# sparsemat/sprs

Hardware: NVIDIA H100
Metric: csr_spmv_f64_gflops (higher is better)
Workload: dtype f64

## Files before the change

sprs_b200/csrc/api.cu:

```cuda

#include <algorithm>
#include <mutex>
#include <vector>

#include <cstdlib>

#include "common.cuh"
#include "ptx.cuh"

namespace {

__global__ void make_policies_kernel(uint64_t* out) {
    out[0] = policy_evict_first();
    out[1] = policy_evict_last();
}

thread_local std::string g_create_error;

template <typename Src, typename Dst>
__global__ void convert_rebase_kernel(const Src* __restrict__ in, Dst* __restrict__ out,
                                      uint64_t n, uint64_t base) {
    const uint64_t i = blockIdx.x * (uint64_t)blockDim.x + threadIdx.x;
    if (i < n) out[i] = (Dst)((uint64_t)in[i] - base);
}
// ... 303 lines not shown
        }
        if ((st = upload_indexlike(ctx, indptr, indptr_bytes, outer + 1, base, m->d_indptr,
                                   m->indptr_bytes, s)) != SPRS_B200_OK)
            break;
        if ((st = upload_indexlike(ctx, indices, index_bytes, nnz, 0, m->d_indices, 4, s)) !=
            SPRS_B200_OK)
            break;
        if (nnz > 0) {
            e = cudaMemcpyAsync(m->d_data, data, nnz * sizeof(double), cudaMemcpyHostToDevice, s);
            if (e != cudaSuccess) {
                sprs_b200_set_error(ctx, cudaGetErrorString(e));
                st = SPRS_B200_ERR_CUDA;
                break;
            }
        }
        if ((st = spmv_prepare(ctx, m, s)) != SPRS_B200_OK) break;
        e = cudaStreamSynchronize(s);
        if (e != cudaSuccess) {
            sprs_b200_set_error(ctx, cudaGetErrorString(e));
            st = SPRS_B200_ERR_CUDA;
        }
    } while (0);
    if (st != SPRS_B200_OK) {
        sprs_b200_csmat_free(m);
        return st;
    }
    *out = m;
    return SPRS_B200_OK;
}

int sprs_b200_csmat_from_device(sprs_b200_ctx* ctx, int storage, uint64_t rows, uint64_t cols,
                                uint64_t nnz, const uint32_t* d_indptr,
                                const uint32_t* d_indices, const double* d_data,
                                sprs_b200_csmat** out) {
    if (!ctx || !out || !d_indptr) return SPRS_B200_ERR_ARGUMENT;
    *out = nullptr;
    if (nnz >= 0xffffffffull || rows > 0xffffffffull || cols > 0xffffffffull)
        SPRS_FAIL(ctx, SPRS_B200_ERR_INDEX_RANGE, "from_device takes u32 arrays only");
    if (((uintptr_t)d_indices | (uintptr_t)d_data) & 15)
        SPRS_FAIL(ctx, SPRS_B200_ERR_ARGUMENT, "device arrays must be 16-byte aligned");
    SPRS_CUDA(ctx, cudaSetDevice(ctx->device));
    auto* m = new sprs_b200_csmat();
    m->ctx = ctx;
    m->storage = storage;
    m->rows = rows;
    m->cols = cols;
    m->nnz = nnz;
    m->outer = storage == SPRS_B200_CSR ? rows : cols;
    m->inner = storage == SPRS_B200_CSR ? cols : rows;
    m->indptr_bytes = 4;
    m->d_indptr = const_cast<uint32_t*>(d_indptr);
    m->d_indices = const_cast<uint32_t*>(d_indices);
    m->d_data = const_cast<double*>(d_data);
    m->owns = false;
    int st = spmv_prepare(ctx, m, ctx->stream);
    if (st == SPRS_B200_OK && cudaStreamSynchronize(ctx->stream) != cudaSuccess) {
        sprs_b200_set_error(ctx, "from_device: partition kernel failed");
        st = SPRS_B200_ERR_CUDA;
    }
    if (st != SPRS_B200_OK) {
        sprs_b200_csmat_free(m);
        return st;
    }
    *out = m;
    return SPRS_B200_OK;
}

int sprs_b200_csmat_free(sprs_b200_csmat* m) {
    if (!m) return SPRS_B200_OK;
    if (m->ctx) cudaSetDevice(m->ctx->device);
    if (m->owns && m->pooled && m->ctx) {
        cudaDeviceSynchronize();
        if (m->d_indptr) cudaFreeAsync(m->d_indptr, m->ctx->stream);
        if (m->d_indices) cudaFreeAsync(m->d_indices, m->ctx->stream);
        if (m->d_data) cudaFreeAsync(m->d_data, m->ctx->stream);
    } else if (m->owns) {
        if (m->d_indptr) cudaFree(m->d_indptr);
        if (m->d_indices) cudaFree(m->d_indices);
        if (m->d_data) cudaFree(m->d_data);
    }
    if (m->d_tile_row) cudaFree(m->d_tile_row);
    if (m->d_tile_k) cudaFree(m->d_tile_k);
    if (m->d_carry) cudaFree(m->d_carry);
    if (m->csr_cache) sprs_b200_csmat_free(m->csr_cache);
    delete m;
    return SPRS_B200_OK;
}

static int csr_of(sprs_b200_ctx* ctx, const sprs_b200_csmat* m, const sprs_b200_csmat** out) {
    if (m->storage == SPRS_B200_CSR) {
        *out = m;
        return SPRS_B200_OK;
    }
    if (!m->csr_cache) {
        sprs_b200_csmat* t = nullptr;
        SPRS_TRY(sprs_b200_csmat_to_other_storage(ctx, m, &t));
        m->csr_cache = t;
    }
    *out = m->csr_cache;
    return SPRS_B200_OK;
}

int sprs_b200_csmat_storage(const sprs_b200_csmat* m) { return m ? m->storage : -1; }
uint64_t sprs_b200_csmat_rows(const sprs_b200_csmat* m) { return m ? m->rows : 0; }
uint64_t sprs_b200_csmat_cols(const sprs_b200_csmat* m) { return m ? m->cols : 0; }
uint64_t sprs_b200_csmat_nnz(const sprs_b200_csmat* m) { return m ? m->nnz : 0; }

int sprs_b200_csmat_download(sprs_b200_ctx* ctx, const sprs_b200_csmat* m, void* indptr,
                             int indptr_bytes, void* indices, int index_bytes, double* data) {
    if (!ctx || !m || !indptr) return SPRS_B200_ERR_ARGUMENT;
    if ((indptr_bytes != 4 && indptr_bytes != 8) || (index_bytes != 4 && index_bytes != 8))
        SPRS_FAIL(ctx, SPRS_B200_ERR_ARGUMENT, "bad index width");
    if (indptr_bytes == 4 && m->nnz > 0xffffffffull)
        SPRS_FAIL(ctx, SPRS_B200_ERR_INDEX_RANGE, "Index type is not large enough for nnz");
    SPRS_CUDA(ctx, cudaSetDevice(ctx->device));
    cudaStream_t s = ctx->stream;
    SPRS_TRY(download_indexlike(ctx, m->d_indptr, m->indptr_bytes, m->outer + 1, indptr,
                                indptr_bytes, s));
    if (m->nnz) {
        if (!indices || !data) return SPRS_B200_ERR_ARGUMENT;
        SPRS_TRY(download_indexlike(ctx, m->d_indices, 4, m->nnz, indices, index_bytes, s));
        SPRS_CUDA(ctx, cudaMemcpyAsync(data, m->d_data, m->nnz * sizeof(double),
                                       cudaMemcpyDeviceToHost, s));
        SPRS_CUDA(ctx, cudaStreamSynchronize(s));
    }
    return SPRS_B200_OK;
}

int sprs_b200_csmat_device_arrays(const sprs_b200_csmat* m, const void** d_indptr,
                                  int* indptr_bytes, const uint32_t** d_indices,
                                  const double** d_data) {
    if (!m) return SPRS_B200_ERR_ARGUMENT;
    if (d_indptr) *d_indptr = m->d_indptr;
    if (indptr_bytes) *indptr_bytes = m->indptr_bytes;
    if (d_indices) *d_indices = m->d_indices;
    if (d_data) *d_data = m->d_data;
    return SPRS_B200_OK;
}

static int finish_triplets(sprs_b200_ctx* ctx, sprs_b200_csmat* t, int st, sprs_b200_csmat** out) {
    if (st == SPRS_B200_OK) st = spmv_prepare(ctx, t, ctx->stream);
    if (st == SPRS_B200_OK && cudaStreamSynchronize(ctx->stream) != cudaSuccess) {
        sprs_b200_set_error(ctx, "from_triplets: kernel failed");
        st = SPRS_B200_ERR_CUDA;
    }
    if (st != SPRS_B200_OK) {
        sprs_b200_csmat_free(t);
        return st;
    }
    *out = t;
    return SPRS_B200_OK;
}

int sprs_b200_csmat_from_triplets_dev(sprs_b200_ctx* ctx, uint64_t rows, uint64_t cols,
                                      uint64_t n, const uint32_t* d_row, const uint32_t* d_col,
                                      const double* d_val, sprs_b200_csmat** out) {
    if (!ctx || !out || (n && (!d_row || !d_col || !d_val))) return SPRS_B200_ERR_ARGUMENT;
    *out = nullptr;
    SPRS_CUDA(ctx, cudaSetDevice(ctx->device));
    auto* t = new sprs_b200_csmat();
    return finish_triplets(ctx, t, triplets_to_csr_launch(ctx, rows, cols, n, d_row, d_col, d_val,
                                                         t, ctx->stream), out);
}

int sprs_b200_csmat_from_triplets(sprs_b200_ctx* ctx, uint64_t rows, uint64_t cols, uint64_t n,
                                  const void* row_inds, const void* col_inds, int index_bytes,
// ... 318 lines not shown
```

sprs_b200/csrc/common.cuh:

```cuda
#pragma once
#include <cuda_runtime.h>

#include <cstdint>
#include <cstdio>
#include <cstring>
#include <string>
#include <vector>

#include "../../include/sprs_b200.h"

constexpr int SPRS_E2E_MAX_CHUNKS = 8;
constexpr int SPRS_E2E_DEFAULT_CHUNKS = 8;

struct sprs_b200_ctx {
    int device = 0;
    int sm_count = 132;
    size_t l2_bytes = 0;
    cudaStream_t stream = nullptr;
    std::string last_error;
    uint64_t launches = 0;
    uint64_t pol_evict_first = 0, pol_evict_last = 0;
    void* h_stage = nullptr;
    size_t h_stage_bytes = 0;
    void* d_scratch[4] = {nullptr, nullptr, nullptr, nullptr};
    size_t d_scratch_bytes[4] = {0, 0, 0, 0};
    cudaStream_t side_stream = nullptr;
    cudaEvent_t ev_fork = nullptr, ev_join = nullptr;
    cudaStream_t copy_stream = nullptr;
    cudaEvent_t ev_chunk[SPRS_E2E_MAX_CHUNKS] = {};
    cudaEvent_t ev_copied = nullptr;
};

struct sprs_b200_csmat {
    sprs_b200_ctx* ctx = nullptr;
    int storage = SPRS_B200_CSR;
    uint64_t rows = 0, cols = 0, nnz = 0;
    uint64_t outer = 0, inner = 0;
    int indptr_bytes = 4;
    void* d_indptr = nullptr;
    uint32_t* d_indices = nullptr;
    double* d_data = nullptr;
    bool owns = true;
    bool pooled = false;
    uint32_t* d_tile_row = nullptr;
    void* d_tile_k = nullptr;
    double* d_carry = nullptr;
    uint64_t n_tiles = 0;
    mutable sprs_b200_csmat* csr_cache = nullptr;
    mutable std::vector<uint64_t> e2e_tiles, e2e_rows;
    mutable std::vector<uint64_t> push_tiles, push_rows;
};

#define SPRS_FAIL(ctx, code, ...)                                  \
    do {                                                           \
        char _buf[512];                                            \
        snprintf(_buf, sizeof(_buf), __VA_ARGS__);                 \
        sprs_b200_set_error((ctx), _buf);                          \
        return (code);                                             \
    } while (0)

#define SPRS_CUDA(ctx, expr)                                                              \
    do {                                                                                  \
        cudaError_t _e = (expr);                                                          \
        if (_e != cudaSuccess)                                                            \
            SPRS_FAIL((ctx), SPRS_B200_ERR_CUDA, "%s failed: %s (%s:%d)", #expr,          \
                      cudaGetErrorString(_e), __FILE__, __LINE__);                        \
    } while (0)

#define SPRS_TRY(expr)                      \
    do {                                    \
        int _s = (expr);                    \
        if (_s != SPRS_B200_OK) return _s;  \
    } while (0)

void sprs_b200_set_error(const sprs_b200_ctx* ctx, const char* msg);

static inline cudaStream_t pick_stream(sprs_b200_ctx*, void* stream) {
    return (cudaStream_t)stream;
}

int ctx_scratch(sprs_b200_ctx* ctx, int i, size_t bytes, void** out);
int ctx_stage(sprs_b200_ctx* ctx, size_t bytes, void** out);

constexpr int SPMV_MAX_TARGETS = 8;
struct SpmvTargets {
    double* p[SPMV_MAX_TARGETS];
    int n;
};

int spmv_prepare(sprs_b200_ctx* ctx, sprs_b200_csmat* m, cudaStream_t s);
int spmv_tile_nnz();
int spmv_launch(sprs_b200_ctx* ctx, const sprs_b200_csmat* m, const double* d_x, double* d_y,
                int accumulate, cudaStream_t s);
int spmv_launch_targets(sprs_b200_ctx* ctx, const sprs_b200_csmat* m, const double* d_x,
                        const SpmvTargets& yt, int accumulate, cudaStream_t s);
int spmv_launch_tile_range(sprs_b200_ctx* ctx, const sprs_b200_csmat* m, const double* d_x,
                           double* d_y, int accumulate, uint64_t t0, uint64_t t1, cudaStream_t s);
int csmat_chunk_table(sprs_b200_ctx* ctx, const sprs_b200_csmat* m, uint64_t n_chunks, bool taper,
                      cudaStream_t s, std::vector<uint64_t>* tiles, std::vector<uint64_t>* rows);
int ctx_side_stream(sprs_b200_ctx* ctx);
int peer_push_launch(sprs_b200_ctx* ctx, const double* src, const SpmvTargets& dst, uint64_t count,
                     cudaStream_t s);
int spmm_rowmaj_launch(sprs_b200_ctx* ctx, const sprs_b200_csmat* m, const double* d_b,
                       uint64_t ldb, uint64_t k, double* d_c, uint64_t ldc, int accumulate,
                       cudaStream_t s);
int triplets_to_csr_launch(sprs_b200_ctx* ctx, uint64_t rows, uint64_t cols, uint64_t n,
                           const uint32_t* d_row, const uint32_t* d_col, const double* d_val,
                           sprs_b200_csmat* out, cudaStream_t s);
int transpose_launch(sprs_b200_ctx* ctx, const sprs_b200_csmat* m, sprs_b200_csmat* out,
                     cudaStream_t s);
int csmat_csr_view(sprs_b200_ctx* ctx, const sprs_b200_csmat* m, const sprs_b200_csmat** out);

#ifdef __CUDACC__
__device__ __forceinline__ uint32_t smem_u32(const void* p) {
    return (uint32_t)__cvta_generic_to_shared(p);
}
__device__ __forceinline__ uint64_t mix64(uint64_t z) {
    z += 0x9E3779B97F4A7C15ull;
    z = (z ^ (z >> 30)) * 0xBF58476D1CE4E5B9ull;
    z = (z ^ (z >> 27)) * 0x94D049BB133111EBull;
    return z ^ (z >> 31);
}
#endif
```

sprs_b200/csrc/spgemm.cu:

```cuda

#include <cstdlib>
#include <vector>

#include "common.cuh"
#include "scan.cuh"

struct sprs_b200_spgemm {
    sprs_b200_ctx* ctx = nullptr;
    const sprs_b200_csmat* a = nullptr;
    const sprs_b200_csmat* b = nullptr;
    uint64_t rows = 0, cols = 0, nnz_c = 0, n_prod = 0;
    uint64_t* d_nprod = nullptr;
    uint32_t* d_cnt = nullptr;
    uint64_t* d_cptr = nullptr;
    uint32_t* d_lists = nullptr;
    uint32_t* d_counters = nullptr;
};

namespace {

constexpr uint32_t EMPTY = 0xffffffffu;
constexpr int NT = 256;
constexpr int WARPS = NT / 32;
constexpr uint32_t SYM_S_MAX = 128, SYM_M_MAX = 8192;
// ... 757 lines not shown
            break;
        }
        const uint32_t *l0 = p->d_lists, *l1 = p->d_lists + rows, *l2 = p->d_lists + 2ull * rows;
        if (h_cnt[0]) {
            sym_small_kernel<<<std::min<unsigned>((h_cnt[0] + WARPS - 1) / WARPS, cap * 4), NT, 0,
                               s>>>(a_ip, a->d_indices, b_ip, b->d_indices, l0, h_cnt[0],
                                    p->d_cnt);
            ctx->launches += 1;
        }
        if (h_cnt[1]) {
            const size_t smem = SYM_M_SLOTS * sizeof(uint32_t);
            cudaFuncSetAttribute(sym_med_kernel, cudaFuncAttributeMaxDynamicSharedMemorySize,
                                 (int)smem);
            sym_med_kernel<<<std::min<unsigned>(h_cnt[1], cap), NT, smem, s>>>(
                a_ip, a->d_indices, b_ip, b->d_indices, p->d_nprod, l1, h_cnt[1], p->d_cnt,
                1);
            ctx->launches += 1;
        }
        if (h_cnt[2]) {
            LargeWorkspace w;
            if ((st = plan_large(ctx, p->cols, h_cnt[2], false, &w, s)) != SPRS_B200_OK) break;
            auto kern = w.smem ? sym_large_kernel<true> : sym_large_kernel<false>;
            if (w.smem)
                cudaFuncSetAttribute(kern, cudaFuncAttributeMaxDynamicSharedMemorySize,
                                     (int)w.smem);
            kern<<<w.grid, SYM_L_NT, w.smem, s>>>(a_ip, a->d_indices, b_ip, b->d_indices, l2,
                                                  h_cnt[2], w.words, w.bitmaps, p->d_cnt, 1,
                                                  p->d_counters + 5);
            ctx->launches += 1;
            cudaStreamSynchronize(s);
            free_large(w);
        }
        if ((st = device_exclusive_scan<uint32_t, uint64_t>(ctx, p->d_cnt, rows, p->d_cptr, s)) !=
            SPRS_B200_OK)
            break;
        if (cudaMemcpyAsync(&p->nnz_c, p->d_cptr + rows, 8, cudaMemcpyDeviceToHost, s) !=
                cudaSuccess ||
            cudaStreamSynchronize(s) != cudaSuccess || cudaGetLastError() != cudaSuccess) {
            sprs_b200_set_error(ctx, "spgemm symbolic: kernel failed");
            st = SPRS_B200_ERR_CUDA;
        }
    } while (0);
    if (st != SPRS_B200_OK) {
        sprs_b200_spgemm_free(p);
        return st;
    }
    *plan = p;
    *nnz_c = p->nnz_c;
    return SPRS_B200_OK;
}

int sprs_b200_spgemm_numeric_dev(sprs_b200_ctx* ctx, sprs_b200_spgemm* p, sprs_b200_csmat** c) {
    if (!ctx || !p || !c) return SPRS_B200_ERR_ARGUMENT;
    *c = nullptr;
    SPRS_CUDA(ctx, cudaSetDevice(ctx->device));
    cudaStream_t s = ctx->stream;
    auto* m = new sprs_b200_csmat();
    m->ctx = ctx;
    m->storage = SPRS_B200_CSR;
    m->rows = p->rows;
    m->cols = p->cols;
    m->nnz = p->nnz_c;
    m->outer = p->rows;
    m->inner = p->cols;
    m->indptr_bytes = p->nnz_c >= 0xffffffffull ? 8 : 4;
    m->pooled = true;
    int st = SPRS_B200_OK;
    do {
        if (cudaMallocAsync(&m->d_indptr, (m->rows + 1) * (size_t)m->indptr_bytes + 16, s) != cudaSuccess ||
            cudaMallocAsync((void**)&m->d_indices, m->nnz * 4 + 16, s) != cudaSuccess ||
            cudaMallocAsync((void**)&m->d_data, m->nnz * 8 + 16, s) != cudaSuccess) {
            sprs_b200_set_error(ctx, "spgemm numeric: cudaMalloc of C failed");
            st = SPRS_B200_ERR_CUDA;
            break;
        }
        if (m->indptr_bytes == 4) {
            widen_kernel<uint64_t, uint32_t><<<grid_for(m->rows + 1), 256, 0, s>>>(
                p->d_cptr, (uint32_t*)m->d_indptr, m->rows + 1);
            ctx->launches += 1;
        } else {
            cudaMemcpyAsync(m->d_indptr, p->d_cptr, (m->rows + 1) * 8, cudaMemcpyDeviceToDevice, s);
        }
        if ((st = run_numeric(ctx, p, m->d_indices, m->d_data, s)) != SPRS_B200_OK) break;
        if ((st = spmv_prepare(ctx, m, s)) != SPRS_B200_OK) break;
        if (cudaStreamSynchronize(s) != cudaSuccess || cudaGetLastError() != cudaSuccess) {
            sprs_b200_set_error(ctx, "spgemm numeric: kernel failed");
            st = SPRS_B200_ERR_CUDA;
        }
    } while (0);
    if (st != SPRS_B200_OK) {
        sprs_b200_csmat_free(m);
        return st;
    }
    *c = m;
    return SPRS_B200_OK;
}

int sprs_b200_spgemm_numeric(sprs_b200_ctx* ctx, sprs_b200_spgemm* p, void* c_indptr,
                             int indptr_bytes, void* c_indices, int index_bytes,
                             double* c_data) {
    if (!ctx || !p || !c_indptr) return SPRS_B200_ERR_ARGUMENT;
    if (p->nnz_c && (!c_indices || !c_data)) return SPRS_B200_ERR_ARGUMENT;
    sprs_b200_csmat* c = nullptr;
    SPRS_TRY(sprs_b200_spgemm_numeric_dev(ctx, p, &c));
    const int st = sprs_b200_csmat_download(ctx, c, c_indptr, indptr_bytes, c_indices,
                                            index_bytes, c_data);
    sprs_b200_csmat_free(c);
    return st;
}

uint64_t sprs_b200_spgemm_nprod(const sprs_b200_spgemm* p) {
    if (!p || !p->d_nprod || p->rows == 0) return 0;
    auto* q = const_cast<sprs_b200_spgemm*>(p);
    if (q->n_prod == 0) {
        std::vector<uint64_t> h(p->rows);
        cudaSetDevice(p->ctx->device);
        if (cudaMemcpy(h.data(), p->d_nprod, p->rows * 8, cudaMemcpyDeviceToHost) == cudaSuccess)
            for (uint64_t v : h) q->n_prod += v;
    }
    return q->n_prod;
}

int sprs_b200_spgemm_free(sprs_b200_spgemm* p) {
    if (!p) return SPRS_B200_OK;
    if (p->ctx) cudaSetDevice(p->ctx->device);
    cudaStream_t s = p->ctx ? p->ctx->stream : nullptr;
    if (p->d_nprod) cudaFreeAsync(p->d_nprod, s);
    if (p->d_cnt) cudaFreeAsync(p->d_cnt, s);
    if (p->d_cptr) cudaFreeAsync(p->d_cptr, s);
    if (p->d_lists) cudaFreeAsync(p->d_lists, s);
    if (p->d_counters) cudaFreeAsync(p->d_counters, s);
    delete p;
    return SPRS_B200_OK;
}

}
```

sprs_b200/csrc/spmv.cu:

```cuda

#include "common.cuh"
#include "ptx.cuh"

#include <cstdlib>

namespace {

constexpr int SPMV_STAGE_ROWS = 66;
constexpr uint32_t SPMV_ROW_COST = 16;

template <typename P>
__global__ void tile_cut_kernel(const P* __restrict__ indptr, uint32_t rows, uint64_t nnz,
                                uint64_t n_tiles, uint32_t w, uint32_t row_cost,
                                uint32_t* __restrict__ tile_row, P* __restrict__ tile_k) {
    const uint64_t t = blockIdx.x * (uint64_t)blockDim.x + threadIdx.x;
    if (t > n_tiles) return;
    if (t == n_tiles) {
        tile_row[t] = rows;
        tile_k[t] = (P)nnz;
        return;
    }
    const uint64_t d = t * (uint64_t)w;
    uint32_t lo = 0, hi = rows;
    while (lo < hi) {
        const uint32_t mid = lo + (hi - lo + 1) / 2;
        if ((uint64_t)indptr[mid] + (uint64_t)row_cost * mid <= d)
            lo = mid;
        else
            hi = mid - 1;
    }
    uint64_t k = d - (uint64_t)row_cost * lo;
    const uint64_t row_end = lo < rows ? (uint64_t)indptr[(size_t)lo + 1] : nnz;
    if (k > row_end) k = row_end;
    tile_row[t] = lo;
    tile_k[t] = (P)k;
}

struct RowSink {
    double* y;
    const SpmvTargets* yt;
    double* carry_slot;
    uint32_t r1;
    int accumulate;
    double* stage;
    uint32_t stage_off;
};
template <bool MULTI>
__device__ __forceinline__ void sink_row(const RowSink& k, uint64_t r, double sum) {
    if (r < k.r1) {
        const double v = k.accumulate ? __dadd_rn(k.y[r], sum) : sum;
        k.y[r] = v;
        if (MULTI) {
#pragma unroll
            if (k.stage) {
                k.stage[(uint32_t)r - k.stage_off] = v;
            } else {
#pragma unroll
                for (int q = 1; q < SPMV_MAX_TARGETS; ++q)
                    if (q < k.yt->n) k.yt->p[q][r] = v;
            }
        }
    } else {
        *k.carry_slot = sum;
    }
}

template <typename P, int G, int U, bool MULTI>
__device__ __forceinline__ void rows_direct(const RowSink& k, const P* __restrict__ indptr,
                                            const uint32_t* __restrict__ indices,
                                            const double* __restrict__ data,
                                            const double* __restrict__ x, P k0, P k1,
                                            uint32_t r0, uint32_t r_last, P b_first,
                                            uint64_t pol_stream, uint64_t polx, int lane) {
    constexpr int NG = 32 / G;
    constexpr unsigned FULL = 0xffffffffu;
    static_assert(G >= 4, "tiny rows have their own sweep: groups start at 4 lanes");
    const int gid = lane / G, gl = lane % G;
    P b = b_first;
    for (uint32_t rbase = r0;; rbase += 31) {
        if (rbase != r0) {
            const uint32_t rr = rbase + lane;
            b = (rr >= rbase && rr <= r_last + 1) ? indptr[rr] : (P)0;
        }
        const int nrows = (r_last - rbase + 1) < 31 ? (int)(r_last - rbase + 1) : 31;
        P ms = b, me = __shfl_down_sync(FULL, b, 1);
        ms = ms > k0 ? ms : k0;
        me = me < k1 ? me : k1;
        if (lane >= nrows || me < ms) me = ms;
        const bool tiny = lane < nrows && (me - ms) <= (P)(2 * U);
        if (__any_sync(FULL, tiny && me > ms)) {
            double acc = 0.0;
#pragma unroll
            for (int st = 0; st < 2; ++st) {
                const P q = ms + (P)(st * U);
                uint32_t c[U];
                double v[U], xv[U];
#pragma unroll
                for (int u = 0; u < U; ++u)
                    c[u] = (tiny && q + (P)u < me) ? ldg_stream_u32(indices + q + (P)u, pol_stream) : 0u;
#pragma unroll
                for (int u = 0; u < U; ++u)
                    v[u] = (tiny && q + (P)u < me) ? ldg_stream_f64(data + q + (P)u, pol_stream) : 0.0;
#pragma unroll
                for (int u = 0; u < U; ++u)
                    xv[u] = (tiny && q + (P)u < me) ? ldg_f64_hint(x + c[u], polx) : 0.0;
#pragma unroll
                for (int u = 0; u < U; ++u)
                    if (tiny && q + (P)u < me) acc = __dadd_rn(acc, __dmul_rn(v[u], xv[u]));
                if (!__any_sync(FULL, tiny && q + (P)U < me)) break;
            }
            if (tiny) sink_row<MULTI>(k, (uint64_t)rbase + lane, acc);
        } else if (tiny) {
            sink_row<MULTI>(k, (uint64_t)rbase + lane, 0.0);
        }
        unsigned todo = __ballot_sync(FULL, lane < nrows && !tiny);
        while (todo) {
            int j = -1;
#pragma unroll
            for (int g = 0; g < NG; ++g) {
                if (todo) {
                    const int jj = __ffs(todo) - 1;
                    todo &= todo - 1;
                    if (gid == g) j = jj;
                }
            }
            const bool valid = j >= 0;
            const int js = valid ? j : 0;
            P s = __shfl_sync(FULL, b, js);
            P e = __shfl_sync(FULL, b, js + 1);
            s = s > k0 ? s : k0;
            e = e < k1 ? e : k1;
            if (!valid || e < s) e = s;
            const bool is_long = (G < 32) && (e - s) > (P)(4 * G * U);
            double acc = 0.0;
            for (P q = s + gl; q < (is_long ? s : e); q += (P)(G * U)) {
                uint32_t c[U];
                double v[U], xv[U];
#pragma unroll
                for (int u = 0; u < U; ++u)
                    c[u] = q + (P)(u * G) < e ? ldg_stream_u32(indices + q + (P)(u * G), pol_stream) : 0u;
#pragma unroll
                for (int u = 0; u < U; ++u)
                    v[u] = q + (P)(u * G) < e ? ldg_stream_f64(data + q + (P)(u * G), pol_stream) : 0.0;
#pragma unroll
                for (int u = 0; u < U; ++u)
                    xv[u] = q + (P)(u * G) < e ? ldg_f64_hint(x + c[u], polx) : 0.0;
#pragma unroll
                for (int u = 0; u < U; ++u)
                    if (q + (P)(u * G) < e) acc = __dadd_rn(acc, __dmul_rn(v[u], xv[u]));
            }
#pragma unroll
            for (int o = G / 2; o > 0; o >>= 1) acc = __dadd_rn(acc, __shfl_xor_sync(FULL, acc, o));
            if (gl == 0 && valid && !is_long) sink_row<MULTI>(k, (uint64_t)rbase + j, acc);
            if (G < 32) {
                unsigned pending = __ballot_sync(FULL, gl == 0 && is_long);
                while (pending) {
                    const int src = __ffs(pending) - 1;
                    pending &= pending - 1;
                    const P qs = __shfl_sync(FULL, s, src), qe = __shfl_sync(FULL, e, src);
                    const int jj = __shfl_sync(FULL, j, src);
                    double a2 = 0.0;
                    for (P q = qs + lane; q < qe; q += (P)(32 * U)) {
                        uint32_t c[U];
                        double v[U], xv[U];
#pragma unroll
                        for (int u = 0; u < U; ++u)
                            c[u] = q + (P)(u * 32) < qe ? ldg_stream_u32(indices + q + (P)(u * 32), pol_stream) : 0u;
#pragma unroll
                        for (int u = 0; u < U; ++u)
                            v[u] = q + (P)(u * 32) < qe ? ldg_stream_f64(data + q + (P)(u * 32), pol_stream) : 0.0;
#pragma unroll
                        for (int u = 0; u < U; ++u)
                            xv[u] = q + (P)(u * 32) < qe ? ldg_f64_hint(x + c[u], polx) : 0.0;
#pragma unroll
                        for (int u = 0; u < U; ++u)
                            if (q + (P)(u * 32) < qe) a2 = __dadd_rn(a2, __dmul_rn(v[u], xv[u]));
                    }
#pragma unroll
                    for (int o = 16; o > 0; o >>= 1) a2 = __dadd_rn(a2, __shfl_xor_sync(FULL, a2, o));
                    if (lane == 0) sink_row<MULTI>(k, (uint64_t)rbase + jj, a2);
                }
            }
        }
        if (r_last - rbase < 31) break;
    }
}

template <typename P, int NWARPS, int MINB, int U, bool MULTI>
__global__ void __launch_bounds__(NWARPS * 32, MINB)
    spmv_rows_kernel(const P* __restrict__ indptr, const uint32_t* __restrict__ indices,
                     const double* __restrict__ data, const uint32_t* __restrict__ tile_row,
                     const P* __restrict__ tile_k, const double* __restrict__ x,
                     const __grid_constant__ SpmvTargets yt,
                     double* __restrict__ carry, uint64_t nnz, uint32_t rows, uint32_t t_begin,
                     uint32_t t_end , int accumulate,
                     uint64_t pol_stream , uint64_t polx ,
                     int stage_rows ) {
    const int lane = threadIdx.x & 31, warp = threadIdx.x >> 5;
    const uint32_t GW = gridDim.x * NWARPS;
    RowSink sink;
    sink.y = yt.p[0];
    sink.yt = &yt;
    sink.accumulate = accumulate;
    sink.stage = nullptr;
    sink.stage_off = 0;
    double* my_stage = nullptr;
    if constexpr (MULTI) {
        __shared__ __align__(16) double stage_all[NWARPS * SPMV_STAGE_ROWS];
        my_stage = stage_all + warp * SPMV_STAGE_ROWS;
    }
    const uint32_t par = MULTI ? (uint32_t)(((uintptr_t)yt.p[1] >> 3) & 1) : 0u;
    uint32_t t = t_begin + blockIdx.x * NWARPS + warp;
    if (t >= t_end) return;
    uint32_t r0 = tile_row[t], r1 = tile_row[t + 1];
    P k0 = tile_k[t], k1 = tile_k[t + 1];
    P b_first = (uint64_t)r0 + lane <= (r1 < rows ? (uint64_t)r1 + 1 : (uint64_t)r1)
                    ? indptr[(size_t)r0 + lane] : (P)0;
    for (;;) {
        const uint32_t tn = t + GW;
        uint32_t r0n = 0, r1n = 0;
        P k0n = 0, k1n = 0;
        if (tn < t_end) {
            r0n = tile_row[tn];
            r1n = tile_row[tn + 1];
            k0n = tile_k[tn];
            k1n = tile_k[tn + 1];
        }
        sink.carry_slot = carry + t;
        sink.r1 = r1;
        if (MULTI && stage_rows) {
            const uint32_t base = (r0 + par) & ~1u;
            const bool fits = r1 > r0 && (r1 + par - base) <= (uint32_t)SPMV_STAGE_ROWS;
            sink.stage = fits ? my_stage : nullptr;
            sink.stage_off = base - par;
            if (fits) {
                if (lane == 0) bulk_wait_group_read0();
                __syncwarp();
            }
        }
        const uint32_t r_last = r1 < rows ? r1 : r1 - 1;
        const uint64_t cnt = k1 - k0, nr = (uint64_t)(r_last - r0) + 1;
#define SPMV_ROWS(G)                                                                            \
    rows_direct<P, G, U, MULTI>(sink, indptr, indices, data, x, k0, k1, r0, r_last, b_first,       \
                             pol_stream, polx, lane)
        if (cnt <= 24 * nr)
            SPMV_ROWS(4);
        else if (cnt <= 48 * nr)
            SPMV_ROWS(8);
        else if (cnt <= 96 * nr)
            SPMV_ROWS(16);
        else
            SPMV_ROWS(32);
#undef SPMV_ROWS
        if (MULTI && sink.stage) {
            fence_proxy_async();
            __syncwarp();
            if (lane == 0) {
                uint32_t lo = r0, hi = r1;
                if ((lo + par) & 1u) {
                    const double v = my_stage[lo - sink.stage_off];
                    for (int q = 1; q < yt.n; ++q) yt.p[q][lo] = v;
                    ++lo;
                }
                if ((hi - lo) & 1u) {
                    --hi;
                    const double v = my_stage[hi - sink.stage_off];
                    for (int q = 1; q < yt.n; ++q) yt.p[q][hi] = v;
                }
                if (hi > lo) {
                    for (int q = 1; q < yt.n; ++q)
                        bulk_s2g(yt.p[q] + lo, my_stage + (lo - sink.stage_off), (hi - lo) * 8u);
                    bulk_commit_group();
                }
            }
            sink.stage = nullptr;
        }
        if (tn >= t_end) break;
        const P b_next = (uint64_t)r0n + lane <= (r1n < rows ? (uint64_t)r1n + 1 : (uint64_t)r1n)
                             ? indptr[(size_t)r0n + lane] : (P)0;
        t = tn;
        r0 = r0n;
        r1 = r1n;
        k0 = k0n;
        k1 = k1n;
        b_first = b_next;
    }
    if (MULTI && stage_rows && lane == 0) bulk_wait_group0();
}

__global__ void spmv_fixup_kernel(const uint32_t* __restrict__ tile_row,
                                  const double* __restrict__ carry, SpmvTargets yt,
                                  uint64_t n_tiles) {
    const uint64_t t = blockIdx.x * (uint64_t)blockDim.x + threadIdx.x;
    if (t + 1 >= n_tiles) return;
    const uint32_t row = tile_row[t + 1];
    if (t > 0 && tile_row[t] == row) return;
    uint64_t lo = t + 1, hi = n_tiles - 1;
    for (uint64_t step = 1; lo + step < hi; step <<= 1) {
        if (tile_row[lo + step + 1] > row) {
            hi = lo + step;
            break;
        }
        lo += step;
    }
    while (lo < hi) {
        const uint64_t mid = lo + (hi - lo) / 2;
        if (tile_row[mid + 1] > row)
            hi = mid;
        else
            lo = mid + 1;
    }
    double sum = carry[t];
#pragma unroll 8
    for (uint64_t u = t + 1; u < lo; ++u) sum = __dadd_rn(sum, carry[u]);
    const double v = __dadd_rn(yt.p[0][row], sum);
#pragma unroll
    for (int q = 0; q < SPMV_MAX_TARGETS; ++q)
        if (q < yt.n) yt.p[q][row] = v;
}

__device__ __forceinline__ void apply_carries_ending_in(const uint32_t* __restrict__ tile_row,
                                                        const double* carry, double* y,
                                                        uint64_t u) {
    const uint32_t row = tile_row[u];
    if (tile_row[u + 1] == row) return;
    uint64_t hi = u, lo = 1;
    for (uint64_t step = 1; step < hi; step <<= 1) {
        if (tile_row[hi - step] < row) {
            lo = hi - step + 1;
            break;
        }
        hi -= step;
    }
    while (lo < hi) {
        const uint64_t mid = lo + (hi - lo) / 2;
        if (tile_row[mid] >= row)
            hi = mid;
        else
            lo = mid + 1;
    }
    double sum = __ldcg(carry + lo - 1);
    for (uint64_t v = lo; v < u; ++v) sum = __dadd_rn(sum, __ldcg(carry + v));
    y[row] = __dadd_rn(__ldcg(y + row), sum);
}

__global__ void spmv_fixup_range_kernel(const uint32_t* __restrict__ tile_row, const double* carry,
                                        double* y, uint64_t u_lo, uint64_t u_hi) {
    const uint64_t u = u_lo + blockIdx.x * (uint64_t)blockDim.x + threadIdx.x;
    if (u >= 1 && u < u_hi) apply_carries_ending_in(tile_row, carry, y, u);
}

struct SpmvVariant {
    int wt, row_cost;
};
SpmvVariant spmv_variant() {
    static SpmvVariant v = [] {
        SpmvVariant d{1024, (int)SPMV_ROW_COST};
        if (const char* e = getenv("SPRS_B200_SPMV_VARIANT")) {
            int a, rc = (int)SPMV_ROW_COST;
            const int got = sscanf(e, "%d,%d", &a, &rc);
            if (got >= 1 && a >= 64 && rc >= 0) d = SpmvVariant{a, rc};
        }
        return d;
    }();
    return v;
}

constexpr int SPMV_NWARPS = 8, SPMV_CTAS_PER_SM = 5, SPMV_LOADS_IN_FLIGHT = 4;

template <typename P>
int launch_variant(sprs_b200_ctx* ctx, const sprs_b200_csmat* m, const double* d_x,
                   const SpmvTargets& yt, int accumulate, uint64_t t0, uint64_t t1,
                   cudaStream_t s) {
    if (m->n_tiles >= 0xffffffffull)
        SPRS_FAIL(ctx, SPRS_B200_ERR_UNSUPPORTED, "spmv: more than 2^32 tiles");
    constexpr int CTAS = SPMV_CTAS_PER_SM, U = SPMV_LOADS_IN_FLIGHT;
    const bool multi = yt.n > 1;
    auto kern = multi ? spmv_rows_kernel<P, SPMV_NWARPS, CTAS, U, true>
                      : spmv_rows_kernel<P, SPMV_NWARPS, CTAS, U, false>;
    static bool configured_flags[64][2] = {};
    bool& configured = configured_flags[ctx->device & 63][multi ? 1 : 0];
    if (!configured) {
        int carve = multi ? 15 : 0;
        if (const char* e = getenv("SPRS_B200_SPMV_CARVEOUT")) carve = atoi(e);
        SPRS_CUDA(ctx, cudaFuncSetAttribute(kern, cudaFuncAttributePreferredSharedMemoryCarveout,
                                            carve));
        configured = true;
    }
    int stage_rows = 0;
    if (multi) {
        stage_rows = yt.n > 2 ? SPMV_STAGE_ROWS : 0;
        if (const char* e = getenv("SPRS_B200_SPMV_PEER_STORES")) {
            if (e[0] == 'd') stage_rows = 0;
            if (e[0] == 't') stage_rows = SPMV_STAGE_ROWS;
        }
        for (int q = 2; q < yt.n; ++q)
            if ((((uintptr_t)yt.p[q] ^ (uintptr_t)yt.p[1]) >> 3) & 1) stage_rows = 0;
    }
    uint64_t grid = (uint64_t)ctx->sm_count * CTAS;
    const uint64_t need = (t1 - t0 + SPMV_NWARPS - 1) / SPMV_NWARPS;
    if (grid > need) grid = need;
    kern<<<(unsigned)grid, SPMV_NWARPS * 32, 0, s>>>((const P*)m->d_indptr, m->d_indices,
                                                     m->d_data, m->d_tile_row, (const P*)m->d_tile_k, d_x, yt,
                                                     m->d_carry,
                                                     m->nnz, (uint32_t)m->rows, (uint32_t)t0,
                                                     (uint32_t)t1, accumulate, ctx->pol_evict_first,
                                                     ctx->pol_evict_last, stage_rows);
    return SPRS_B200_OK;
}

int check_spmv_args(sprs_b200_ctx* ctx, const sprs_b200_csmat* m) {
    if (m->storage != SPRS_B200_CSR)
        SPRS_FAIL(ctx, SPRS_B200_ERR_STORAGE, "Storage mismatch: spmv needs a CSR mirror");
    if (!m->d_tile_row) SPRS_FAIL(ctx, SPRS_B200_ERR_ARGUMENT, "csmat has no SpMV partition");
    return SPRS_B200_OK;
}

}

int spmv_tile_nnz() { return spmv_variant().wt; }

int spmv_prepare(sprs_b200_ctx* ctx, sprs_b200_csmat* m, cudaStream_t s) {
    if (m->storage != SPRS_B200_CSR) return SPRS_B200_OK;
    const uint32_t w = (uint32_t)spmv_tile_nnz();
    const uint32_t row_cost = (uint32_t)spmv_variant().row_cost;
    const uint64_t total = m->nnz + (uint64_t)row_cost * m->rows;
    m->n_tiles = total == 0 ? 1 : (total + w - 1) / w;
    SPRS_CUDA(ctx, cudaMalloc((void**)&m->d_tile_row, (m->n_tiles + 1) * sizeof(uint32_t)));
    SPRS_CUDA(ctx, cudaMalloc((void**)&m->d_tile_k, (m->n_tiles + 1) * (size_t)m->indptr_bytes));
    SPRS_CUDA(ctx, cudaMalloc((void**)&m->d_carry, m->n_tiles * sizeof(double)));
    const uint64_t n = m->n_tiles + 1;
    const unsigned grid = (unsigned)((n + 255) / 256);
    if (m->indptr_bytes == 4)
        tile_cut_kernel<uint32_t><<<grid, 256, 0, s>>>((const uint32_t*)m->d_indptr, (uint32_t)m->rows,
                                                       m->nnz, m->n_tiles, w, row_cost, m->d_tile_row,
                                                       (uint32_t*)m->d_tile_k);
    else
        tile_cut_kernel<uint64_t><<<grid, 256, 0, s>>>((const uint64_t*)m->d_indptr, (uint32_t)m->rows,
                                                       m->nnz, m->n_tiles, w, row_cost, m->d_tile_row,
                                                       (uint64_t*)m->d_tile_k);
    ctx->launches += 1;
    SPRS_CUDA(ctx, cudaGetLastError());
    return SPRS_B200_OK;
}

int spmv_launch_targets(sprs_b200_ctx* ctx, const sprs_b200_csmat* m, const double* d_x,
                        const SpmvTargets& yt, int accumulate, cudaStream_t s) {
    SPRS_TRY(check_spmv_args(ctx, m));
    if (m->rows == 0) return SPRS_B200_OK;
    if (m->indptr_bytes == 4)
        SPRS_TRY(launch_variant<uint32_t>(ctx, m, d_x, yt, accumulate, 0, m->n_tiles, s));
    else
        SPRS_TRY(launch_variant<uint64_t>(ctx, m, d_x, yt, accumulate, 0, m->n_tiles, s));
    ctx->launches += 1;
    if (m->n_tiles > 1) {
        const unsigned fgrid = (unsigned)((m->n_tiles - 1 + 255) / 256);
        spmv_fixup_kernel<<<fgrid, 256, 0, s>>>(m->d_tile_row, m->d_carry, yt, m->n_tiles);
        ctx->launches += 1;
    }
    SPRS_CUDA(ctx, cudaGetLastError());
    return SPRS_B200_OK;
}

int spmv_launch_tile_range(sprs_b200_ctx* ctx, const sprs_b200_csmat* m, const double* d_x,
                           double* d_y, int accumulate, uint64_t t0, uint64_t t1,
                           cudaStream_t s) {
    SPRS_TRY(check_spmv_args(ctx, m));
    if (t1 > m->n_tiles || t0 >= t1) SPRS_FAIL(ctx, SPRS_B200_ERR_ARGUMENT, "bad tile range");
    SpmvTargets yt;
    yt.n = 1;
    yt.p[0] = d_y;
    for (int q = 1; q < SPMV_MAX_TARGETS; ++q) yt.p[q] = nullptr;
    if (m->indptr_bytes == 4)
        SPRS_TRY(launch_variant<uint32_t>(ctx, m, d_x, yt, accumulate, t0, t1, s));
    else
        SPRS_TRY(launch_variant<uint64_t>(ctx, m, d_x, yt, accumulate, t0, t1, s));
    spmv_fixup_range_kernel<<<(unsigned)((t1 - t0 + 255) / 256), 256, 0, s>>>(
        m->d_tile_row, m->d_carry, d_y, t0, t1);
    ctx->launches += 2;
    SPRS_CUDA(ctx, cudaGetLastError());
    return SPRS_B200_OK;
}

int spmv_launch(sprs_b200_ctx* ctx, const sprs_b200_csmat* m, const double* d_x, double* d_y,
                int accumulate, cudaStream_t s) {
    SpmvTargets yt;
    yt.n = 1;
    yt.p[0] = d_y;
    for (int q = 1; q < SPMV_MAX_TARGETS; ++q) yt.p[q] = nullptr;
    return spmv_launch_targets(ctx, m, d_x, yt, accumulate, s);
}
```

Before: 208.5.

## Cache hottest x columns in shared memory for SpMV with tagged indices

```diff
diff --git a/sprs_b200/csrc/api.cu b/sprs_b200/csrc/api.cu
--- a/sprs_b200/csrc/api.cu
+++ b/sprs_b200/csrc/api.cu
@@ -409,6 +409,8 @@
     if (m->d_tile_row) cudaFree(m->d_tile_row);
     if (m->d_tile_k) cudaFree(m->d_tile_k);
     if (m->d_carry) cudaFree(m->d_carry);
+    if (m->d_hot_col) cudaFree(m->d_hot_col);
+    if (m->d_hot_idx) cudaFree(m->d_hot_idx);
     if (m->csr_cache) sprs_b200_csmat_free(m->csr_cache);
     delete m;
     return SPRS_B200_OK;
diff --git a/sprs_b200/csrc/common.cuh b/sprs_b200/csrc/common.cuh
--- a/sprs_b200/csrc/common.cuh
+++ b/sprs_b200/csrc/common.cuh
@@ -46,6 +46,9 @@
     void* d_tile_k = nullptr;
     double* d_carry = nullptr;
     uint64_t n_tiles = 0;
+    uint32_t* d_hot_col = nullptr;
+    uint32_t* d_hot_idx = nullptr;
+    uint32_t n_hot = 0;
     mutable sprs_b200_csmat* csr_cache = nullptr;
     mutable std::vector<uint64_t> e2e_tiles, e2e_rows;
     mutable std::vector<uint64_t> push_tiles, push_rows;
@@ -88,7 +91,7 @@
     int n;
 };
 
-int spmv_prepare(sprs_b200_ctx* ctx, sprs_b200_csmat* m, cudaStream_t s);
+int spmv_prepare(sprs_b200_ctx* ctx, sprs_b200_csmat* m, cudaStream_t s, bool hot_set = true);
 int spmv_tile_nnz();
 int spmv_launch(sprs_b200_ctx* ctx, const sprs_b200_csmat* m, const double* d_x, double* d_y,
                 int accumulate, cudaStream_t s);
diff --git a/sprs_b200/csrc/spgemm.cu b/sprs_b200/csrc/spgemm.cu
--- a/sprs_b200/csrc/spgemm.cu
+++ b/sprs_b200/csrc/spgemm.cu
@@ -863,7 +863,7 @@
             cudaMemcpyAsync(m->d_indptr, p->d_cptr, (m->rows + 1) * 8, cudaMemcpyDeviceToDevice, s);
         }
         if ((st = run_numeric(ctx, p, m->d_indices, m->d_data, s)) != SPRS_B200_OK) break;
-        if ((st = spmv_prepare(ctx, m, s)) != SPRS_B200_OK) break;
+        if ((st = spmv_prepare(ctx, m, s, false)) != SPRS_B200_OK) break;
         if (cudaStreamSynchronize(s) != cudaSuccess || cudaGetLastError() != cudaSuccess) {
             sprs_b200_set_error(ctx, "spgemm numeric: kernel failed");
             st = SPRS_B200_ERR_CUDA;
diff --git a/sprs_b200/csrc/spmv.cu b/sprs_b200/csrc/spmv.cu
--- a/sprs_b200/csrc/spmv.cu
+++ b/sprs_b200/csrc/spmv.cu
@@ -1,7 +1,9 @@
 
 #include "common.cuh"
 #include "ptx.cuh"
-
+#include "scan.cuh"
+
+#include <algorithm>
 #include <cstdlib>
 
 namespace {
@@ -65,11 +67,19 @@
     }
 }
 
-template <typename P, int G, int U, bool MULTI>
+constexpr uint32_t HOT_TAG = 0x80000000u;
+template <bool HOT>
+__device__ __forceinline__ double gather_x(const double* __restrict__ x, const double* hot,
+                                           uint32_t c, uint64_t polx) {
+    if (HOT && (c & HOT_TAG)) return hot[c & ~HOT_TAG];
+    return ldg_f64_hint(x + c, polx);
+}
+
+template <typename P, int G, int U, bool MULTI, bool HOT>
 __device__ __forceinline__ void rows_direct(const RowSink& k, const P* __restrict__ indptr,
                                             const uint32_t* __restrict__ indices,
                                             const double* __restrict__ data,
-                                            const double* __restrict__ x, P k0, P k1,
+                                            const double* __restrict__ x, const double* hot, P k0, P k1,
                                             uint32_t r0, uint32_t r_last, P b_first,
                                             uint64_t pol_stream, uint64_t polx, int lane) {
     constexpr int NG = 32 / G;
@@ -103,7 +113,7 @@
                     v[u] = (tiny && q + (P)u < me) ? ldg_stream_f64(data + q + (P)u, pol_stream) : 0.0;
 #pragma unroll
                 for (int u = 0; u < U; ++u)
-                    xv[u] = (tiny && q + (P)u < me) ? ldg_f64_hint(x + c[u], polx) : 0.0;
+                    xv[u] = (tiny && q + (P)u < me) ? gather_x<HOT>(x, hot, c[u], polx) : 0.0;
 #pragma unroll
                 for (int u = 0; u < U; ++u)
                     if (tiny && q + (P)u < me) acc = __dadd_rn(acc, __dmul_rn(v[u], xv[u]));
@@ -144,7 +154,7 @@
                     v[u] = q + (P)(u * G) < e ? ldg_stream_f64(data + q + (P)(u * G), pol_stream) : 0.0;
 #pragma unroll
                 for (int u = 0; u < U; ++u)
-                    xv[u] = q + (P)(u * G) < e ? ldg_f64_hint(x + c[u], polx) : 0.0;
+                    xv[u] = q + (P)(u * G) < e ? gather_x<HOT>(x, hot, c[u], polx) : 0.0;
 #pragma unroll
                 for (int u = 0; u < U; ++u)
                     if (q + (P)(u * G) < e) acc = __dadd_rn(acc, __dmul_rn(v[u], xv[u]));
@@ -171,7 +181,7 @@
                             v[u] = q + (P)(u * 32) < qe ? ldg_stream_f64(data + q + (P)(u * 32), pol_stream) : 0.0;
 #pragma unroll
                         for (int u = 0; u < U; ++u)
-                            xv[u] = q + (P)(u * 32) < qe ? ldg_f64_hint(x + c[u], polx) : 0.0;
+                            xv[u] = q + (P)(u * 32) < qe ? gather_x<HOT>(x, hot, c[u], polx) : 0.0;
 #pragma unroll
                         for (int u = 0; u < U; ++u)
                             if (q + (P)(u * 32) < qe) a2 = __dadd_rn(a2, __dmul_rn(v[u], xv[u]));
@@ -186,7 +196,7 @@
     }
 }
 
-template <typename P, int NWARPS, int MINB, int U, bool MULTI>
+template <typename P, int NWARPS, int MINB, int U, bool MULTI, bool HOT>
 __global__ void __launch_bounds__(NWARPS * 32, MINB)
     spmv_rows_kernel(const P* __restrict__ indptr, const uint32_t* __restrict__ indices,
                      const double* __restrict__ data, const uint32_t* __restrict__ tile_row,
@@ -195,8 +205,16 @@
                      double* __restrict__ carry, uint64_t nnz, uint32_t rows, uint32_t t_begin,
                      uint32_t t_end , int accumulate,
                      uint64_t pol_stream , uint64_t polx ,
-                     int stage_rows ) {
+                     int stage_rows ,
+                     const uint32_t* __restrict__ hot_col ,
+                     uint32_t n_hot) {
     const int lane = threadIdx.x & 31, warp = threadIdx.x >> 5;
+    extern __shared__ __align__(16) double hot_x[];
+    if constexpr (HOT) {
+        for (uint32_t q = threadIdx.x; q < n_hot; q += NWARPS * 32)
+            hot_x[q] = ldg_f64_hint(x + hot_col[q], polx);
+        __syncthreads();
+    }
     const uint32_t GW = gridDim.x * NWARPS;
     RowSink sink;
     sink.y = yt.p[0];
@@ -241,8 +259,8 @@
         const uint32_t r_last = r1 < rows ? r1 : r1 - 1;
         const uint64_t cnt = k1 - k0, nr = (uint64_t)(r_last - r0) + 1;
 #define SPMV_ROWS(G)                                                                            \
-    rows_direct<P, G, U, MULTI>(sink, indptr, indices, data, x, k0, k1, r0, r_last, b_first,       \
-                             pol_stream, polx, lane)
+    rows_direct<P, G, U, MULTI, HOT>(sink, indptr, indices, data, x, hot_x, k0, k1, r0, r_last,   \
+                                     b_first, pol_stream, polx, lane)
         if (cnt <= 24 * nr)
             SPMV_ROWS(4);
         else if (cnt <= 48 * nr)
@@ -368,21 +386,62 @@
 
 constexpr int SPMV_NWARPS = 8, SPMV_CTAS_PER_SM = 5, SPMV_LOADS_IN_FLIGHT = 4;
 
+constexpr int SPMV_HOT_NWARPS = 32, SPMV_HOT_CTAS_PER_SM = 1;
+constexpr uint32_t SPMV_HOT_SLOTS = 24576;
+constexpr uint32_t SPMV_HOT_MAX_SLOTS = 26624;
+constexpr uint64_t SPMV_HOT_MIN_NNZ = 1ull << 25;
+constexpr double SPMV_HOT_MIN_SHARE = 0.10;
+
+struct SpmvHot {
+    uint32_t k;
+    bool forced;
+};
+SpmvHot spmv_hot() {
+    static SpmvHot h = [] {
+        SpmvHot d{SPMV_HOT_SLOTS, false};
+        const char* e = getenv("SPRS_B200_SPMV_HOT");
+        if (e && strcmp(e, "auto") != 0) {
+            const long k = atol(e);
+            d = SpmvHot{(uint32_t)(k < 0 ? 0 : k > (long)SPMV_HOT_MAX_SLOTS ? SPMV_HOT_MAX_SLOTS : k), true};
+        }
+        return d;
+    }();
+    return h;
+}
+
+template <typename P, bool MULTI, bool HOT>
+auto* spmv_kernel() {
+    constexpr int U = SPMV_LOADS_IN_FLIGHT;
+    if constexpr (HOT)
+        return spmv_rows_kernel<P, SPMV_HOT_NWARPS, SPMV_HOT_CTAS_PER_SM, U, MULTI, true>;
+    else
+        return spmv_rows_kernel<P, SPMV_NWARPS, SPMV_CTAS_PER_SM, U, MULTI, false>;
+}
+
 template <typename P>
 int launch_variant(sprs_b200_ctx* ctx, const sprs_b200_csmat* m, const double* d_x,
                    const SpmvTargets& yt, int accumulate, uint64_t t0, uint64_t t1,
                    cudaStream_t s) {
     if (m->n_tiles >= 0xffffffffull)
         SPRS_FAIL(ctx, SPRS_B200_ERR_UNSUPPORTED, "spmv: more than 2^32 tiles");
-    constexpr int CTAS = SPMV_CTAS_PER_SM, U = SPMV_LOADS_IN_FLIGHT;
-    const bool multi = yt.n > 1;
-    auto kern = multi ? spmv_rows_kernel<P, SPMV_NWARPS, CTAS, U, true>
-                      : spmv_rows_kernel<P, SPMV_NWARPS, CTAS, U, false>;
-    static bool configured_flags[64][2] = {};
-    bool& configured = configured_flags[ctx->device & 63][multi ? 1 : 0];
+    const bool multi = yt.n > 1, hot = m->n_hot > 0;
+    auto kern = hot ? (multi ? spmv_kernel<P, true, true>() : spmv_kernel<P, false, true>())
+                    : (multi ? spmv_kernel<P, true, false>() : spmv_kernel<P, false, false>());
+    const int nwarps = hot ? SPMV_HOT_NWARPS : SPMV_NWARPS;
+    const int ctas = hot ? SPMV_HOT_CTAS_PER_SM : SPMV_CTAS_PER_SM;
+    static bool configured_flags[64][4] = {};
+    bool& configured = configured_flags[ctx->device & 63][(multi ? 1 : 0) + (hot ? 2 : 0)];
     if (!configured) {
-        int carve = multi ? 15 : 0;
-        if (const char* e = getenv("SPRS_B200_SPMV_CARVEOUT")) carve = atoi(e);
+        int carve;
+        if (hot) {
+            const int dyn = (int)(spmv_hot().k * sizeof(double));
+            const int per_cta = dyn + (multi ? nwarps * SPMV_STAGE_ROWS * 8 : 0) + 1024;
+            SPRS_CUDA(ctx, cudaFuncSetAttribute(kern, cudaFuncAttributeMaxDynamicSharedMemorySize, dyn));
+            carve = (int)((100ull * ctas * per_cta + 228 * 1024 - 1) / (228 * 1024));
+        } else {
+            carve = multi ? 15 : 0;
+            if (const char* e = getenv("SPRS_B200_SPMV_CARVEOUT")) carve = atoi(e);
+        }
         SPRS_CUDA(ctx, cudaFuncSetAttribute(kern, cudaFuncAttributePreferredSharedMemoryCarveout,
                                             carve));
         configured = true;
@@ -397,16 +456,166 @@
         for (int q = 2; q < yt.n; ++q)
             if ((((uintptr_t)yt.p[q] ^ (uintptr_t)yt.p[1]) >> 3) & 1) stage_rows = 0;
     }
-    uint64_t grid = (uint64_t)ctx->sm_count * CTAS;
-    const uint64_t need = (t1 - t0 + SPMV_NWARPS - 1) / SPMV_NWARPS;
+    uint64_t grid = (uint64_t)ctx->sm_count * ctas;
+    const uint64_t need = (t1 - t0 + nwarps - 1) / nwarps;
     if (grid > need) grid = need;
-    kern<<<(unsigned)grid, SPMV_NWARPS * 32, 0, s>>>((const P*)m->d_indptr, m->d_indices,
-                                                     m->d_data, m->d_tile_row, (const P*)m->d_tile_k, d_x, yt,
-                                                     m->d_carry,
-                                                     m->nnz, (uint32_t)m->rows, (uint32_t)t0,
-                                                     (uint32_t)t1, accumulate, ctx->pol_evict_first,
-                                                     ctx->pol_evict_last, stage_rows);
+    const size_t smem = hot ? m->n_hot * sizeof(double) : 0;
+    kern<<<(unsigned)grid, nwarps * 32, smem, s>>>((const P*)m->d_indptr,
+                                                   hot ? m->d_hot_idx : m->d_indices,
+                                                   m->d_data, m->d_tile_row, (const P*)m->d_tile_k, d_x, yt,
+                                                   m->d_carry,
+                                                   m->nnz, (uint32_t)m->rows, (uint32_t)t0,
+                                                   (uint32_t)t1, accumulate, ctx->pol_evict_first,
+                                                   ctx->pol_evict_last, stage_rows, m->d_hot_col,
+                                                   m->n_hot);
     return SPRS_B200_OK;
+}
+
+__device__ __forceinline__ void add_aggregated(uint32_t* counts, uint32_t key, unsigned active) {
+    const unsigned peers = __match_any_sync(active, key);
+    if ((int)(threadIdx.x & 31) == __ffs(peers) - 1) atomicAdd(counts + key, (uint32_t)__popc(peers));
+}
+
+__global__ void hot_count_kernel(const uint32_t* __restrict__ indices, uint64_t nnz,
+                                 uint32_t* __restrict__ counts) {
+    const uint64_t stride = (uint64_t)gridDim.x * blockDim.x;
+    for (uint64_t base = blockIdx.x * (uint64_t)blockDim.x + (threadIdx.x & ~31u); base < nnz;
+         base += stride) {
+        const uint64_t i = base + (threadIdx.x & 31);
+        const bool valid = i < nnz;
+        const unsigned active = __ballot_sync(0xffffffffu, valid);
+        if (valid) add_aggregated(counts, indices[i], active);
+    }
+}
+
+__global__ void hot_count_hist_kernel(const uint32_t* __restrict__ counts, uint32_t cols,
+                                      uint32_t hi, uint32_t* __restrict__ hist) {
+    const uint64_t stride = (uint64_t)gridDim.x * blockDim.x;
+    for (uint64_t base = blockIdx.x * (uint64_t)blockDim.x + (threadIdx.x & ~31u); base < cols;
+         base += stride) {
+        const uint64_t i = base + (threadIdx.x & 31);
+        const uint32_t c = i < cols ? counts[i] : 0u;
+        const bool take = c > 0 && (hi == ~0u || (c >> 16) == hi);
+        const unsigned active = __ballot_sync(0xffffffffu, take);
+        if (take) add_aggregated(hist, hi == ~0u ? c >> 16 : c & 0xffffu, active);
+    }
+}
+
+__global__ void hot_flag_kernel(const uint32_t* __restrict__ counts, uint32_t cols, uint32_t thr,
+                                const uint32_t* __restrict__ tie_rank, uint32_t ties,
+                                uint8_t* __restrict__ flag) {
+    const uint64_t i = blockIdx.x * (uint64_t)blockDim.x + threadIdx.x;
+    if (i >= cols) return;
+    const uint32_t c = counts[i];
+    flag[i] = tie_rank ? (c > thr || (c == thr && tie_rank[i] < ties)) : c == thr;
+}
+
+__global__ void hot_map_kernel(uint32_t* __restrict__ counts_map, uint32_t cols,
+                               const uint8_t* __restrict__ sel, const uint32_t* __restrict__ slot,
+                               uint32_t* __restrict__ hot_col, unsigned long long* hot_nnz) {
+    const uint64_t i = blockIdx.x * (uint64_t)blockDim.x + threadIdx.x;
+    if (i >= cols) return;
+    if (sel[i]) {
+        const uint32_t q = slot[i];
+        atomicAdd(hot_nnz, (unsigned long long)counts_map[i]);
+        hot_col[q] = (uint32_t)i;
+        counts_map[i] = HOT_TAG | q;
+    } else {
+        counts_map[i] = (uint32_t)i;
+    }
+}
+
+__global__ void hot_tag_kernel(const uint32_t* __restrict__ indices, uint64_t nnz,
+                               const uint32_t* __restrict__ map, uint32_t* __restrict__ tagged) {
+    const uint64_t stride = (uint64_t)gridDim.x * blockDim.x;
+    for (uint64_t i = blockIdx.x * (uint64_t)blockDim.x + threadIdx.x; i < nnz; i += stride)
+        tagged[i] = map[indices[i]];
+}
+
+int spmv_prepare_hot(sprs_b200_ctx* ctx, sprs_b200_csmat* m, cudaStream_t s) {
+    const SpmvHot cfg = spmv_hot();
+    if (cfg.k == 0 || m->nnz == 0 || m->cols == 0 || m->cols >= HOT_TAG) return SPRS_B200_OK;
+    if (!cfg.forced && m->nnz < SPMV_HOT_MIN_NNZ) return SPRS_B200_OK;
+    const uint32_t cols = (uint32_t)m->cols;
+    uint32_t *counts = nullptr, *hist = nullptr, *slot = nullptr, *hot_col = nullptr,
+             *hot_idx = nullptr;
+    uint8_t* flag = nullptr;
+    unsigned long long* d_hot_nnz = nullptr;
+    const unsigned grid_nnz =
+        (unsigned)std::min<uint64_t>((m->nnz + 255) / 256, (uint64_t)ctx->sm_count * 16);
+    const unsigned grid_cols = (unsigned)((cols + 255) / 256);
+    auto build = [&]() -> int {
+        if (cudaMalloc((void**)&counts, cols * sizeof(uint32_t)) != cudaSuccess ||
+            cudaMalloc((void**)&hist, 65536 * sizeof(uint32_t)) != cudaSuccess ||
+            cudaMalloc((void**)&flag, cols) != cudaSuccess ||
+            cudaMalloc((void**)&slot, (cols + 1ull) * sizeof(uint32_t)) != cudaSuccess ||
+            cudaMalloc((void**)&d_hot_nnz, sizeof(unsigned long long)) != cudaSuccess)
+            return SPRS_B200_OK;
+        SPRS_CUDA(ctx, cudaMemsetAsync(counts, 0, cols * sizeof(uint32_t), s));
+        SPRS_CUDA(ctx, cudaMemsetAsync(hist, 0, 65536 * sizeof(uint32_t), s));
+        SPRS_CUDA(ctx, cudaMemsetAsync(d_hot_nnz, 0, sizeof(unsigned long long), s));
+        hot_count_kernel<<<grid_nnz, 256, 0, s>>>(m->d_indices, m->nnz, counts);
+        hot_count_hist_kernel<<<grid_cols, 256, 0, s>>>(counts, cols, ~0u, hist);
+        ctx->launches += 2;
+        std::vector<uint32_t> h(65536);
+        SPRS_CUDA(ctx, cudaMemcpyAsync(h.data(), hist, 65536 * sizeof(uint32_t),
+                                       cudaMemcpyDeviceToHost, s));
+        SPRS_CUDA(ctx, cudaStreamSynchronize(s));
+        uint64_t above = 0, referenced = 0;
+        for (uint32_t b = 0; b < 65536; ++b) referenced += h[b];
+        uint32_t k = cfg.k, thr = 1, ties = 0xffffffffu;
+        if (referenced > k) {
+            uint32_t bhi = 65535;
+            while (above + h[bhi] < k) above += h[bhi--];
+            SPRS_CUDA(ctx, cudaMemsetAsync(hist, 0, 65536 * sizeof(uint32_t), s));
+            hot_count_hist_kernel<<<grid_cols, 256, 0, s>>>(counts, cols, bhi, hist);
+            ctx->launches += 1;
+            SPRS_CUDA(ctx, cudaMemcpyAsync(h.data(), hist, 65536 * sizeof(uint32_t),
+                                           cudaMemcpyDeviceToHost, s));
+            SPRS_CUDA(ctx, cudaStreamSynchronize(s));
+            uint32_t blo = 65535;
+            while (above + h[blo] < k) above += h[blo--];
+            thr = (bhi << 16) | blo;
+            ties = k - (uint32_t)above;
+        } else {
+            k = (uint32_t)referenced;
+        }
+        hot_flag_kernel<<<grid_cols, 256, 0, s>>>(counts, cols, thr, nullptr, 0, flag);
+        ctx->launches += 1;
+        SPRS_TRY((device_exclusive_scan<uint8_t, uint32_t>(ctx, flag, cols, slot, s)));
+        hot_flag_kernel<<<grid_cols, 256, 0, s>>>(counts, cols, thr, slot, ties, flag);
+        ctx->launches += 1;
+        SPRS_TRY((device_exclusive_scan<uint8_t, uint32_t>(ctx, flag, cols, slot, s)));
+        if (cudaMalloc((void**)&hot_col, k * sizeof(uint32_t)) != cudaSuccess) return SPRS_B200_OK;
+        hot_map_kernel<<<grid_cols, 256, 0, s>>>(counts, cols, flag, slot, hot_col, d_hot_nnz);
+        ctx->launches += 1;
+        unsigned long long hot_nnz = 0;
+        SPRS_CUDA(ctx, cudaMemcpyAsync(&hot_nnz, d_hot_nnz, sizeof(hot_nnz), cudaMemcpyDeviceToHost, s));
+        SPRS_CUDA(ctx, cudaStreamSynchronize(s));
+        if (!cfg.forced && (double)hot_nnz < SPMV_HOT_MIN_SHARE * (double)m->nnz) return SPRS_B200_OK;
+        if (cudaMalloc((void**)&hot_idx, m->nnz * sizeof(uint32_t) + 16) != cudaSuccess)
+            return SPRS_B200_OK;
+        hot_tag_kernel<<<grid_nnz, 256, 0, s>>>(m->d_indices, m->nnz, counts, hot_idx);
+        ctx->launches += 1;
+        SPRS_CUDA(ctx, cudaStreamSynchronize(s));
+        SPRS_CUDA(ctx, cudaGetLastError());
+        m->d_hot_col = hot_col;
+        m->d_hot_idx = hot_idx;
+        m->n_hot = k;
+        return SPRS_B200_OK;
+    };
+    const int st = build();
+    if (m->n_hot == 0) {
+        cudaGetLastError();
+        if (hot_col) cudaFree(hot_col);
+        if (hot_idx) cudaFree(hot_idx);
+    }
+    if (counts) cudaFree(counts);
+    if (hist) cudaFree(hist);
+    if (flag) cudaFree(flag);
+    if (slot) cudaFree(slot);
+    if (d_hot_nnz) cudaFree(d_hot_nnz);
+    return st;
 }
 
 int check_spmv_args(sprs_b200_ctx* ctx, const sprs_b200_csmat* m) {
@@ -420,7 +629,7 @@
 
 int spmv_tile_nnz() { return spmv_variant().wt; }
 
-int spmv_prepare(sprs_b200_ctx* ctx, sprs_b200_csmat* m, cudaStream_t s) {
+int spmv_prepare(sprs_b200_ctx* ctx, sprs_b200_csmat* m, cudaStream_t s, bool hot_set) {
     if (m->storage != SPRS_B200_CSR) return SPRS_B200_OK;
     const uint32_t w = (uint32_t)spmv_tile_nnz();
     const uint32_t row_cost = (uint32_t)spmv_variant().row_cost;
@@ -441,6 +650,7 @@
                                                        (uint64_t*)m->d_tile_k);
     ctx->launches += 1;
     SPRS_CUDA(ctx, cudaGetLastError());
+    if (hot_set) SPRS_TRY(spmv_prepare_hot(ctx, m, s));
     return SPRS_B200_OK;
 }
 
```

New measurement: 248.1, median of 6. 1.19x the previous value.
